# Schaudge/cellranger

Measured on AMD Instinct MI355X. Metric: M reads/sec barcode-correct+UMI-count, higher is better.
Workload: dtype u32/u64 integer keys; f64 posterior

## Files before the change

### cellranger_amd/csrc/dedup.hip

```cpp
#include "block_utils.h"
#include "common.h"

int cr_scan_small(crgpu_ctx *ctx, uint32_t *d_data, uint64_t n, uint32_t *d_total_out);
int cr_partition_by_owner(crgpu_ctx *ctx, const uint64_t *d_in, uint64_t *d_out, uint64_t n, uint32_t sh_bc,
                          uint32_t n_ranks, const uint32_t *bounds, uint64_t *counts_out);

#define NONE32 0xFFFFFFFFu

struct crgpu_counts {
    uint64_t n_triplets = 0, n_molecules = 0;
    uint32_t *d_bc = nullptr, *d_feature = nullptr, *d_count = nullptr;
    uint64_t *d_mkeys = nullptr;
    uint32_t *d_mreads = nullptr;
    uint32_t *d_corr_reads = nullptr;
    uint32_t *d_filt_reads = nullptr;
    int32_t *d_mprobe = nullptr;
    uint32_t *d_back = nullptr;
    uint32_t n_back = 0;
    uint32_t n_canon = 0;
    KeyLayout layout;
    bool pt_valid = false;
    uint32_t pt_n_probes = 0;
    uint64_t n_pt = 0;
    uint32_t *d_pt_bc = nullptr, *d_pt_probe = nullptr, *d_pt_count = nullptr;
// ... 512 lines not shown
        }
#undef CR_BUILD_KEYS
        CR_HIP(ctx, hipGetLastError());
    }
    unsigned long long h = 0;
    CR_TRY(crgpu_memcpy_d2h(ctx, &h, d_n, sizeof(h)));
    if (d_vals_out) {
        uint32_t stalled = 0;
        CR_TRY(crgpu_memcpy_d2h(ctx, &stalled, d_lb_abort, sizeof(stalled)));
        if (stalled) {
            ctx->ghist.valid = false;
            return cr_fail(ctx, CRGPU_EHIP, "crgpu_build_keys: the look-back of the order-preserving compaction stalled (watchdog); "
                                            "nothing was hung, the keys of this call are incomplete");
        }
    }
    if (d_fwd) {
        uint32_t unknown = 0;
        CR_TRY(crgpu_memcpy_d2h(ctx, &unknown, d_unknown, sizeof(unknown)));
        if (unknown) {
            ctx->ghist.valid = false;
            return cr_fail(ctx, CRGPU_ESTATE, "crgpu_build_keys: %u records carry a barcode that has no read in the VALID / CORRECTED tables "
                           "(CRGPU_OPT_DENSE_BARCODE_KEYS needs the tables of the whole well before the first key is built)", unknown);
        }
    }
    *n_keys_out = h;
    ctx->ghist.n = append ? n_before + h : h;
    return CRGPU_OK;
}

extern "C" int crgpu_build_keys_dev(crgpu_ctx *ctx, const crgpu_records *recs, uint64_t *d_keys_out,
                                    uint64_t *n_keys_out) {
    if (!ctx) return CRGPU_EINVAL;
    CR_ENTER(ctx);
    return build_keys_impl(ctx, recs, d_keys_out, nullptr, n_keys_out);
}

extern "C" int crgpu_partition_keys_dev(crgpu_ctx *ctx, const uint64_t *d_keys, uint64_t n, uint32_t n_ranks,
                                        const uint32_t *bounds, uint64_t *d_keys_out, uint64_t *counts_out) {
    if (!ctx || !counts_out) return CRGPU_EINVAL;
    CR_ENTER(ctx);
    CR_REQUIRE(ctx, ctx->layout.set, CRGPU_ESTATE, "crgpu_partition_keys: call crgpu_set_key_layout first");
    CR_REQUIRE(ctx, n == 0 || (d_keys && d_keys_out), CRGPU_EINVAL, "crgpu_partition_keys: NULL buffer");
    cr_invalidate(ctx);
    CR_TRY(cr_dense_ensure(ctx));
    return cr_partition_by_owner(ctx, d_keys, d_keys_out, n, ctx->layout.sh_bc(), n_ranks, bounds, counts_out);
}

extern "C" int crgpu_balanced_bounds(crgpu_ctx *ctx, uint32_t n_ranks, uint32_t *bounds_out) {
    if (!ctx || !bounds_out) return CRGPU_EINVAL;
    CR_ENTER(ctx);
    CR_REQUIRE(ctx, ctx->canon_set, CRGPU_ESTATE, "crgpu_balanced_bounds: no whitelist set");
    CR_REQUIRE(ctx, n_ranks >= 1 && n_ranks <= 256, CRGPU_EINVAL, "crgpu_balanced_bounds: n_ranks must be 1..256");
    const uint32_t W = ctx->n_canon;
    std::vector<uint64_t> tot(W, 0);
    std::vector<uint32_t> tmp(W);
    for (int l = 0; l < CRGPU_MAX_LIB; l++) {
        if (!ctx->wl[l].set) continue;
        for (int which = 0; which < 2; which++) {
            CR_TRY(crgpu_memcpy_d2h(ctx, tmp.data(), which ? ctx->wl[l].d_corrected : ctx->wl[l].d_valid, sizeof(uint32_t) * W));
            for (uint32_t r = 0; r < W; r++) tot[r] += tmp[r];
        }
    }
    uint64_t total = 0;
    for (uint32_t r = 0; r < W; r++) total += tot[r];
    bounds_out[0] = 0;
    uint64_t acc = 0;
    uint32_t r = 0;
    for (uint32_t k = 1; k < n_ranks; k++) {
        const uint64_t want = total * k / n_ranks;
        while (r < W && acc + tot[r] <= want) acc += tot[r++];
        bounds_out[k] = r;
    }
    bounds_out[n_ranks] = W;
    return CRGPU_OK;
}

#define CP_BLOCK 256
#ifndef CP_ITEMS
#define CP_ITEMS 8
#endif
#define CP_ROUND (CP_BLOCK * CP_ITEMS)
#define CP_WAVES (CP_BLOCK / 64)

template <typename Flag>
__global__ __launch_bounds__(CP_BLOCK) void k_cp_count(Flag flag, uint64_t n, uint64_t tile, uint32_t *__restrict__ block_counts) {
    __shared__ uint32_t ws[CP_WAVES];
    const uint64_t lo = (uint64_t)blockIdx.x * tile;
    const uint64_t hi = lo + tile < n ? lo + tile : n;
    uint32_t c = 0;
    for (uint64_t base = lo; base < hi; base += CP_ROUND) {
        bool f[CP_ITEMS];
#pragma unroll
        for (int j = 0; j < CP_ITEMS; j++) {
            const uint64_t i = base + (uint64_t)j * CP_BLOCK + threadIdx.x;
            f[j] = flag(i < hi ? i : hi - 1);
        }
#pragma unroll
        for (int j = 0; j < CP_ITEMS; j++) {
            const uint64_t i = base + (uint64_t)j * CP_BLOCK + threadIdx.x;
            c += (f[j] && i < hi) ? 1u : 0u;
        }
    }
#pragma unroll
    for (int d = 32; d >= 1; d >>= 1) c += __shfl_xor(c, d);
    if ((threadIdx.x & 63u) == 0) ws[threadIdx.x >> 6] = c;
    __syncthreads();
    if (threadIdx.x == 0) {
        uint32_t t = 0;
        for (int w = 0; w < CP_WAVES; w++) t += ws[w];
        block_counts[blockIdx.x] = t;
    }
}

template <typename Flag, typename Emit>
__global__ __launch_bounds__(CP_BLOCK) void k_cp_write(Flag flag, Emit emit, uint64_t n, uint64_t tile,
                                                       const uint32_t *__restrict__ block_offs) {
    __shared__ uint32_t ws[CP_ITEMS * CP_WAVES];
    __shared__ uint32_t round_total;
    const uint32_t lane = threadIdx.x & 63u, wave = threadIdx.x >> 6;
    const uint64_t lo = (uint64_t)blockIdx.x * tile;
    const uint64_t hi = lo + tile < n ? lo + tile : n;
    uint32_t run = block_offs[blockIdx.x];
    for (uint64_t base = lo; base < hi; base += CP_ROUND) {
        bool f[CP_ITEMS];
        typename Emit::Pre pre[CP_ITEMS];
#pragma unroll
        for (int j = 0; j < CP_ITEMS; j++) {
            const uint64_t i = base + (uint64_t)j * CP_BLOCK + threadIdx.x;
            f[j] = flag(i < hi ? i : hi - 1);
            pre[j] = emit.pre(i < hi ? i : hi - 1);
        }
        uint32_t below[CP_ITEMS];
#pragma unroll
        for (int j = 0; j < CP_ITEMS; j++) {
            const uint64_t i = base + (uint64_t)j * CP_BLOCK + threadIdx.x;
            f[j] = f[j] && i < hi;
            const unsigned long long m = __ballot(f[j]);
            below[j] = (uint32_t)__popcll(m & ((1ull << lane) - 1ull));
            if (lane == 0) ws[j * CP_WAVES + wave] = (uint32_t)__popcll(m);
        }
        __syncthreads();
        if (threadIdx.x < CP_ITEMS * CP_WAVES) {
            const uint32_t v = ws[threadIdx.x];
            uint32_t x = v;
#pragma unroll
            for (int d = 1; d < CP_ITEMS * CP_WAVES; d <<= 1) {
                const uint32_t y = __shfl_up(x, d);
                if (threadIdx.x >= (uint32_t)d) x += y;
            }
            ws[threadIdx.x] = x - v;
            if (threadIdx.x == CP_ITEMS * CP_WAVES - 1) round_total = x;
        }
        __syncthreads();
#pragma unroll
        for (int j = 0; j < CP_ITEMS; j++) {
            const uint64_t i = base + (uint64_t)j * CP_BLOCK + threadIdx.x;
            if (f[j]) emit(i, run + ws[j * CP_WAVES + wave] + below[j], pre[j]);
        }
        run += round_total;
        __syncthreads();
    }
}

static uint32_t cp_blocks(uint64_t n, uint64_t *tile_out) {
    uint64_t nb = (n + CP_ROUND * 4 - 1) / (CP_ROUND * 4);
    if (nb < 1) nb = 1;
    if (nb > 4096) nb = 4096;
    uint64_t tile = (n + nb - 1) / nb;
    tile = (tile + CP_ROUND - 1) / CP_ROUND * CP_ROUND;
    nb = (n + tile - 1) / tile;
    if (nb < 1) nb = 1;
    *tile_out = tile;
    return (uint32_t)nb;
}

template <typename Flag, typename Emit>
static int compact(crgpu_ctx *ctx, Flag flag, Emit emit, uint64_t n, uint32_t *d_block, uint32_t *d_total_out) {
    uint64_t tile;
    const uint32_t nb = cp_blocks(n, &tile);
    hipLaunchKernelGGL(k_cp_count<Flag>, dim3(nb), dim3(CP_BLOCK), 0, ctx->stream, flag, n, tile, d_block);
    CR_TRY(cr_scan_small(ctx, d_block, nb, d_total_out));
    hipLaunchKernelGGL((k_cp_write<Flag, Emit>), dim3(nb), dim3(CP_BLOCK), 0, ctx->stream, flag, emit, n, tile, d_block);
    CR_HIP(ctx, hipGetLastError());
    return CRGPU_OK;
}

#define ST_CORRECTED 1u
#define ST_LOW 2u
__device__ __forceinline__ uint32_t st_inc1(uint32_t s) { return s >> 2; }
__device__ __forceinline__ void st_or(uint16_t *st, uint64_t k, uint32_t bits) {
    atomicOr(reinterpret_cast<uint32_t *>(st) + (k >> 1), bits << (16u * (uint32_t)(k & 1u)));
}
__device__ __forceinline__ void move_reads(uint32_t *corr, uint16_t *st, uint32_t *inc_all, uint32_t *minidx, uint64_t k,
                                           uint32_t target, uint32_t my_cnt) {
    corr[k] = target;
    st_or(st, k, ST_CORRECTED);
    atomicAdd(reinterpret_cast<uint32_t *>(st) + (target >> 1), 4u << (16u * (target & 1u)));
    atomicAdd(&inc_all[target], my_cnt);
    atomicMin(&minidx[target], (uint32_t)k);
}
__device__ __forceinline__ uint32_t rep_source(uint32_t min_raw, uint32_t K, uint32_t sK) {
    return (min_raw != 0xFFFFFFFFu && (min_raw < K || (sK & ST_CORRECTED))) ? min_raw : 0xFFFFFFFFu;
}

struct TargetFilter {
    const uint8_t *on_target;
    uint32_t n_features, sh_feat, bits_feat;
    uint64_t min_reads;
    __device__ __forceinline__ bool filtered(uint64_t key, uint32_t read_count, bool low) const {
        if (!min_reads) return false;
        const uint32_t f = (uint32_t)((key >> sh_feat) & lowmask(bits_feat));
        return f < n_features && on_target[f] != 0 && (uint64_t)read_count < min_reads && !low;
    }
};
struct MolFlag {
    const uint16_t *st;
    __device__ __forceinline__ bool operator()(uint64_t k) const {
        const uint32_t s = st[k];
        const bool landed = !(s & ST_CORRECTED) | (st_inc1(s) > 0u);
        return landed & !(s & ST_LOW);
    }
};
struct MolFlagTargeted {
    const uint16_t *st;
    const uint64_t *ukey;
    const uint32_t *upos, *inc_all;
    uint64_t n_keys, n_dist;
    TargetFilter tf;
    __device__ __forceinline__ bool operator()(uint64_t k) const {
        const uint32_t s = st[k];
        const bool landed = !(s & ST_CORRECTED) | (st_inc1(s) > 0u);
        if (!landed || (s & ST_LOW)) return false;
        const uint32_t end = k + 1 < n_dist ? upos[k + 1] : (uint32_t)n_keys;
        const uint32_t rc = ((s & ST_CORRECTED) ? 0u : end - upos[k]) + (st_inc1(s) ? inc_all[k] : 0u);
        return !tf.filtered(ukey[k], rc, false);
    }
};
struct EmitMol {
    const uint64_t *ukey;
    const uint32_t *upos, *inc_all, *minidx;
    const uint16_t *st;
    uint64_t n_keys, n_dist;
    uint64_t *mkeys;
    uint32_t *mreads;
    const uint32_t *rep_read = nullptr;
    const int32_t *probe = nullptr;
    int32_t *mprobe = nullptr;
    struct Pre {
        uint64_t key;
        uint32_t p0, p1, s;
    };
    __device__ __forceinline__ Pre pre(uint64_t k) const {
        Pre p;
        p.key = ukey[k];
        p.p0 = upos[k];
        p.p1 = upos[k + 1 < n_dist ? k + 1 : k];
        p.s = st[k];
        return p;
    }
    __device__ __forceinline__ Pre pre_own(uint64_t k) const {
        Pre p;
        p.key = ukey[k];
        p.p0 = upos[k];
        p.p1 = 0u;
        p.s = st[k];
        return p;
    }
    __device__ __forceinline__ void operator()(uint64_t k, uint32_t o, const Pre &p) const {
        uint32_t inc = 0u, mi = NONE32;
        if (st_inc1(p.s)) {
            inc = inc_all[k];
            mi = rep_source(minidx[k], (uint32_t)k, p.s);
        }
        const uint64_t bit = (mi != NONE32 ? ukey[mi] : p.key) & 1ull;
        mkeys[o] = (p.key & ~1ull) | bit;
        const uint32_t end = k + 1 < n_dist ? p.p1 : (uint32_t)n_keys;
        const uint32_t cnt = end - p.p0;
        mreads[o] = ((p.s & ST_CORRECTED) ? 0u : cnt) + inc;
        if (mprobe) mprobe[o] = probe[rep_read[mi != NONE32 ? mi : (uint32_t)k]];
    }
};

__device__ __forceinline__ bool rl_is_head(uint64_t key, uint64_t &carry_key, bool &carry_valid, uint32_t shift, uint32_t lane) {
    uint64_t left = __shfl_up(key, 1);
    if (lane == 0) left = carry_key;
    const bool head = (lane == 0 && !carry_valid) || (key >> shift) != (left >> shift);
    carry_key = __shfl(key, 63);
    carry_valid = true;
    return head;
}

__global__ __launch_bounds__(CP_BLOCK) void k_rl_count(const uint64_t *__restrict__ keys, const uint32_t shift, const uint64_t n,
                                                       const uint64_t tile, uint32_t *__restrict__ block_counts) {
    __shared__ uint32_t ws[CP_WAVES];
    const uint32_t lane = threadIdx.x & 63u, wave = threadIdx.x >> 6;
    const uint64_t lo = (uint64_t)blockIdx.x * tile;
    const uint64_t hi = lo + tile < n ? lo + tile : n;
    uint32_t c = 0;
    for (uint64_t base = lo; base < hi; base += CP_ROUND) {
        uint64_t key[CP_ITEMS];
        const uint64_t w0 = base + (uint64_t)wave * (64u * CP_ITEMS);
        const uint64_t wb = w0 > 0 ? (w0 - 1 < n ? w0 - 1 : n - 1) : 0;
        uint64_t carry_key = keys[wb];
        bool carry_valid = w0 > 0;
#pragma unroll
        for (int j = 0; j < CP_ITEMS; j++) {
            const uint64_t i = w0 + (uint64_t)j * 64 + lane;
            key[j] = keys[i < hi ? i : hi - 1];
        }
#pragma unroll
        for (int j = 0; j < CP_ITEMS; j++) {
            const uint64_t i = w0 + (uint64_t)j * 64 + lane;
            const bool head = rl_is_head(key[j], carry_key, carry_valid, shift, lane);
            c += (head && i < hi) ? 1u : 0u;
        }
    }
#pragma unroll
    for (int d = 32; d >= 1; d >>= 1) c += __shfl_xor(c, d);
    if (lane == 0) ws[wave] = c;
    __syncthreads();
    if (threadIdx.x == 0) {
        uint32_t t = 0;
        for (int w = 0; w < CP_WAVES; w++) t += ws[w];
        block_counts[blockIdx.x] = t;
    }
}

__global__ __launch_bounds__(CP_BLOCK) void k_rl_write(const uint64_t *__restrict__ keys, const uint32_t shift, const uint64_t n,
                                                       const uint64_t tile, const uint32_t *__restrict__ block_offs,
                                                       uint64_t *__restrict__ ukey, uint32_t *__restrict__ upos) {
    __shared__ uint32_t ws[CP_ITEMS * CP_WAVES];
    __shared__ uint32_t round_total;
    const uint32_t lane = threadIdx.x & 63u, wave = threadIdx.x >> 6;
    const uint64_t lo = (uint64_t)blockIdx.x * tile;
    const uint64_t hi = lo + tile < n ? lo + tile : n;
    uint32_t run = block_offs[blockIdx.x];
    for (uint64_t base = lo; base < hi; base += CP_ROUND) {
        uint64_t key[CP_ITEMS];
        bool f[CP_ITEMS];
        uint32_t below[CP_ITEMS];
        const uint64_t w0 = base + (uint64_t)wave * (64u * CP_ITEMS);
        const uint64_t wb = w0 > 0 ? (w0 - 1 < n ? w0 - 1 : n - 1) : 0;
        uint64_t carry_key = keys[wb];
        bool carry_valid = w0 > 0;
#pragma unroll
        for (int j = 0; j < CP_ITEMS; j++) {
            const uint64_t i = w0 + (uint64_t)j * 64 + lane;
            key[j] = keys[i < hi ? i : hi - 1];
        }
#pragma unroll
        for (int j = 0; j < CP_ITEMS; j++) {
            const uint64_t i = w0 + (uint64_t)j * 64 + lane;
            f[j] = rl_is_head(key[j], carry_key, carry_valid, shift, lane) && i < hi;
            const unsigned long long m = __ballot(f[j]);
            below[j] = (uint32_t)__popcll(m & ((1ull << lane) - 1ull));
            if (lane == 0) ws[wave * CP_ITEMS + j] = (uint32_t)__popcll(m);
        }
        __syncthreads();
        if (threadIdx.x < CP_ITEMS * CP_WAVES) {
            const uint32_t v = ws[threadIdx.x];
            uint32_t x = v;
#pragma unroll
            for (int d = 1; d < CP_ITEMS * CP_WAVES; d <<= 1) {
                const uint32_t y = __shfl_up(x, d);
                if (threadIdx.x >= (uint32_t)d) x += y;
            }
            ws[threadIdx.x] = x - v;
            if (threadIdx.x == CP_ITEMS * CP_WAVES - 1) round_total = x;
        }
        __syncthreads();
#pragma unroll
        for (int j = 0; j < CP_ITEMS; j++)
            if (f[j]) {
                const uint32_t o = run + ws[wave * CP_ITEMS + j] + below[j];
                ukey[o] = key[j];
                upos[o] = (uint32_t)(w0 + (uint64_t)j * 64 + lane);
            }
        run += round_total;
        __syncthreads();
    }
}

static int run_lengths(crgpu_ctx *ctx, const uint64_t *keys, uint32_t shift, uint64_t n, uint64_t *ukey, uint32_t *upos,
                       uint32_t *d_block, uint32_t *d_total_out, bool counts_ready = false) {
    uint64_t tile;
    const uint32_t nb = cp_blocks(n, &tile);
    if (!counts_ready)
        hipLaunchKernelGGL(k_rl_count, dim3(nb), dim3(CP_BLOCK), 0, ctx->stream, keys, shift, n, tile, d_block);
    else
        ctx->rl_counts_from_finish++;
    CR_TRY(cr_scan_small(ctx, d_block, nb, d_total_out));
    hipLaunchKernelGGL(k_rl_write, dim3(nb), dim3(CP_BLOCK), 0, ctx->stream, keys, shift, n, tile, d_block, ukey, upos);
    CR_HIP(ctx, hipGetLastError());
    return CRGPU_OK;
}

struct MtCarry {
    uint64_t prefix;
    bool has_mol;
    bool valid;
};

template <typename Flag>
__device__ __forceinline__ MtCarry mt_carry_from_memory(const Flag &flag, const uint64_t *__restrict__ ukey, uint32_t sh_feat,
                                                        uint64_t nd, uint64_t i0) {
    MtCarry c{0ull, false, false};
    if (i0 == 0 || i0 >= nd) return c;
    c.valid = true;
    uint64_t p = i0 - 1;
    c.prefix = ukey[p] >> sh_feat;
    c.has_mol = flag(p);
    while (!c.has_mol && p > 0) {
        p--;
        if ((ukey[p] >> sh_feat) != c.prefix) break;
        c.has_mol = flag(p);
    }
    return c;
}

__device__ __forceinline__ bool mt_opens_triplet(bool is_mol, uint64_t key, uint32_t sh_feat, uint32_t lane, MtCarry &carry) {
    const uint64_t prefix = key >> sh_feat;
    const uint64_t left = __shfl_up(prefix, 1);
    const unsigned long long starts = __ballot(lane == 0 || prefix != left), mols = __ballot(is_mol);
    const unsigned long long upto = ~0ull >> (63u - lane);
    const uint32_t rs = 63u - (uint32_t)__clzll((long long)(starts & upto));
    const unsigned long long between = (upto >> 1) & ~((1ull << rs) - 1ull);
    const uint64_t prefix0 = __shfl(prefix, 0);
    const bool carried = carry.valid && carry.prefix == prefix0 && carry.has_mol;
    const bool open = (mols & between) == 0ull && !(rs == 0u && carried);
    const uint32_t rs_last = 63u - (uint32_t)__clzll((long long)starts);
    const bool last_has = (mols >> rs_last) != 0ull || (rs_last == 0u && carried);
    carry.prefix = __shfl(prefix, 63);
    carry.has_mol = last_has;
    carry.valid = true;
    return is_mol && open;
}

#define MT_WAVE_SPAN (64u * CP_ITEMS)
template <typename Flag>
__global__ __launch_bounds__(CP_BLOCK) void k_mt_count(const Flag flag, const uint64_t *__restrict__ ukey, const uint32_t sh_feat,
                                                       const uint64_t nd, const uint64_t tile, uint32_t *__restrict__ mol_counts,
                                                       uint32_t *__restrict__ head_counts) {
    __shared__ uint32_t ws[2 * CP_WAVES];
    const uint32_t lane = threadIdx.x & 63u, wave = threadIdx.x >> 6;
    const uint64_t lo = (uint64_t)blockIdx.x * tile;
    const uint64_t hi = lo + tile < nd ? lo + tile : nd;
    uint32_t cm = 0, ch = 0;
    for (uint64_t base = lo; base < hi; base += CP_ROUND) {
        bool f[CP_ITEMS];
        uint64_t key[CP_ITEMS];
        const uint64_t w0 = base + (uint64_t)wave * MT_WAVE_SPAN;
#pragma unroll
        for (int j = 0; j < CP_ITEMS; j++) {
            const uint64_t i = w0 + (uint64_t)j * 64 + lane;
            const uint64_t ic = i < hi ? i : hi - 1;
            f[j] = flag(ic);
            key[j] = ukey[ic];
        }
        MtCarry carry = mt_carry_from_memory(flag, ukey, sh_feat, nd, w0);
#pragma unroll
        for (int j = 0; j < CP_ITEMS; j++) {
            const uint64_t i = w0 + (uint64_t)j * 64 + lane;
            const bool m = f[j] && i < hi;
            const bool h = mt_opens_triplet(m, key[j], sh_feat, lane, carry);
            cm += m ? 1u : 0u;
            ch += h ? 1u : 0u;
        }
    }
#pragma unroll
    for (int d = 32; d >= 1; d >>= 1) {
        cm += __shfl_xor(cm, d);
        ch += __shfl_xor(ch, d);
    }
    if (lane == 0) {
        ws[wave] = cm;
        ws[CP_WAVES + wave] = ch;
    }
    __syncthreads();
    if (threadIdx.x == 0) {
        uint32_t tm = 0, th = 0;
        for (int w = 0; w < CP_WAVES; w++) {
            tm += ws[w];
            th += ws[CP_WAVES + w];
        }
        mol_counts[blockIdx.x] = tm;
        head_counts[blockIdx.x] = th;
    }
}

template <typename Flag>
__global__ __launch_bounds__(CP_BLOCK) void k_mt_write(const Flag flag, const EmitMol emit, const uint32_t sh_bc, const uint32_t sh_feat,
                                                       const uint32_t bits_feat, const uint64_t nd, const uint64_t tile,
                                                       const uint32_t *__restrict__ mol_offs, const uint32_t *__restrict__ head_offs,
                                                       uint32_t *__restrict__ tbc, uint32_t *__restrict__ tfeat,
                                                       uint32_t *__restrict__ tpos, const uint32_t *__restrict__ back) {
    __shared__ uint32_t ws[CP_ITEMS * CP_WAVES];
    __shared__ uint32_t round_total;
    const uint32_t lane = threadIdx.x & 63u, wave = threadIdx.x >> 6;
    const uint64_t lo = (uint64_t)blockIdx.x * tile;
    const uint64_t hi = lo + tile < nd ? lo + tile : nd;
    uint32_t run_m = mol_offs[blockIdx.x], run_h = head_offs[blockIdx.x];
    for (uint64_t base = lo; base < hi; base += CP_ROUND) {
        bool f[CP_ITEMS], h[CP_ITEMS];
        EmitMol::Pre pre[CP_ITEMS];
        const uint64_t w0 = base + (uint64_t)wave * MT_WAVE_SPAN;
#pragma unroll
        for (int j = 0; j < CP_ITEMS; j++) {
            const uint64_t i = w0 + (uint64_t)j * 64 + lane;
            const uint64_t ic = i < hi ? i : hi - 1;
            f[j] = flag(ic);
            pre[j] = emit.pre_own(ic);
        }
        {
            const uint64_t il = w0 + (uint64_t)MT_WAVE_SPAN;
            uint32_t after = emit.upos[il < nd ? il : nd - 1];
#pragma unroll
            for (int j = CP_ITEMS - 1; j >= 0; j--) {
                uint32_t nx = __shfl_down(pre[j].p0, 1);
                if (lane == 63u) nx = after;
                pre[j].p1 = nx;
                after = __shfl(pre[j].p0, 0);
            }
        }
        MtCarry carry = mt_carry_from_memory(flag, emit.ukey, sh_feat, nd, w0);
        uint32_t below_m[CP_ITEMS], below_h[CP_ITEMS];
#pragma unroll
        for (int j = 0; j < CP_ITEMS; j++) {
            const uint64_t i = w0 + (uint64_t)j * 64 + lane;
            f[j] = f[j] && i < hi;
            h[j] = mt_opens_triplet(f[j], pre[j].key, sh_feat, lane, carry);
            const unsigned long long mm = __ballot(f[j]), mh = __ballot(h[j]);
            const unsigned long long lt = (1ull << lane) - 1ull;
            below_m[j] = (uint32_t)__popcll(mm & lt);
            below_h[j] = (uint32_t)__popcll(mh & lt);
            if (lane == 0) ws[wave * CP_ITEMS + j] = (uint32_t)__popcll(mm) | ((uint32_t)__popcll(mh) << 16);
        }
        __syncthreads();
        if (threadIdx.x < CP_ITEMS * CP_WAVES) {
            const uint32_t v = ws[threadIdx.x];
            uint32_t x = v;
#pragma unroll
            for (int d = 1; d < CP_ITEMS * CP_WAVES; d <<= 1) {
                const uint32_t y = __shfl_up(x, d);
                if (threadIdx.x >= (uint32_t)d) x += y;
            }
            ws[threadIdx.x] = x - v;
            if (threadIdx.x == CP_ITEMS * CP_WAVES - 1) round_total = x;
        }
        __syncthreads();
#pragma unroll
        for (int j = 0; j < CP_ITEMS; j++)
            if (f[j]) {
                const uint64_t i = w0 + (uint64_t)j * 64 + lane;
                const uint32_t w = ws[wave * CP_ITEMS + j];
                const uint32_t o = run_m + (w & 0xFFFFu) + below_m[j];
                emit(i, o, pre[j]);
                if (h[j]) {
                    const uint32_t t = run_h + (w >> 16) + below_h[j];
                    const uint32_t bcf = (uint32_t)(pre[j].key >> sh_bc);
                    tbc[t] = back ? back[bcf] : bcf;
                    tfeat[t] = (uint32_t)((pre[j].key >> sh_feat) & lowmask(bits_feat));
                    tpos[t] = o;
                }
            }
        run_m += round_total & 0xFFFFu;
        run_h += round_total >> 16;
        __syncthreads();
    }
}

__global__ __launch_bounds__(256) void k_trip_counts(const uint32_t *__restrict__ tpos, uint64_t nt, uint64_t nm,
                                                     uint32_t *__restrict__ cnt) {
    const uint64_t stride = (uint64_t)gridDim.x * blockDim.x;
    for (uint64_t t = (uint64_t)blockIdx.x * blockDim.x + threadIdx.x; t < nt; t += stride)
        cnt[t] = (t + 1 < nt ? tpos[t + 1] : (uint32_t)nm) - tpos[t];
}

__device__ __forceinline__ void segment_bounds(const uint64_t *__restrict__ ukey, uint64_t nd, uint64_t k, uint32_t shift,
                                               uint64_t &s, uint64_t &e) {
    const uint64_t pre = ukey[k] >> shift;
    uint64_t lo = k, step = 1;
    while (lo >= step && (ukey[lo - step] >> shift) == pre) {
        lo -= step;
        step <<= 1;
    }
    uint64_t a = lo >= step ? lo - step + 1 : 0, b = lo;
    while (a < b) {
        const uint64_t mid = (a + b) >> 1;
        if ((ukey[mid] >> shift) == pre) b = mid; else a = mid + 1;
    }
    s = a;
    uint64_t hi = k;
    step = 1;
    while (hi + step < nd && (ukey[hi + step] >> shift) == pre) {
        hi += step;
        step <<= 1;
    }
    a = hi;
    b = hi + step < nd ? hi + step - 1 : nd - 1;
    while (a < b) {
        const uint64_t mid = (a + b + 1) >> 1;
        if ((ukey[mid] >> shift) == pre) a = mid; else b = mid - 1;
    }
    e = a + 1;
}

__device__ __forceinline__ uint32_t run_count(const uint32_t *__restrict__ upos, uint64_t nd, uint64_t n_keys, uint64_t k) {
    const uint32_t end = k + 1 < nd ? upos[k + 1] : (uint32_t)n_keys;
    return end - upos[k];
}

#include "umi_correct.h"

__device__ __forceinline__ uint64_t group_id(const KL &kl, uint64_t key) {
    const uint64_t umi = (key >> kl.sh_umi) & lowmask(kl.bits_umi);
    const uint64_t lib = (key >> kl.sh_lib) & lowmask(kl.bits_lib + kl.bits_ulen);
    const uint64_t bc = key >> kl.sh_bc;
    return ((bc << (kl.bits_lib + kl.bits_ulen)) | lib) << kl.bits_umi | umi;
}
__device__ __forceinline__ uint32_t group_hash(uint64_t g) {
    g ^= g >> 33;
    g *= 0xff51afd7ed558ccdull;
    g ^= g >> 33;
    g *= 0xc4ceb9fe1a85ec53ull;
    g ^= g >> 33;
    return (uint32_t)g;
}

#define LF_TILE 8192u
#define LF_ENTRY_BITS 18u
#define LF_WORDS (1u << (LF_ENTRY_BITS - 4u))
__device__ __forceinline__ uint64_t mix64(uint64_t g) {
    g ^= g >> 33;
    g *= 0xff51afd7ed558ccdull;
    g ^= g >> 33;
    g *= 0xc4ceb9fe1a85ec53ull;
    g ^= g >> 33;
    return g;
}
#define LF_THREADS 1024u
#define LF_BATCH 4
#define LS_HASH_BITS 32u
__device__ __forceinline__ void lf_note(uint32_t *bm, uint32_t e) {
    const uint32_t sh = (e & 15u) * 2u;
    const uint32_t old = atomicOr(&bm[e >> 4], 1u << sh);
    if ((old >> sh) & 1u) atomicOr(&bm[e >> 4], 2u << sh);
}
__device__ __forceinline__ bool lf_again(const uint32_t *bm, uint32_t e) { return (bm[e >> 4] >> ((e & 15u) * 2u + 1u)) & 1u; }
__global__ __launch_bounds__(LF_THREADS) void k_group_candidates(const KL kl, const uint64_t *__restrict__ ukey, uint64_t nd,
                                                                 uint8_t *__restrict__ cand) {
// ... 563 lines not shown
                                   s_in_tmp ? ht_b.as<uint32_t>() : h_b.as<uint32_t>(),
                                   s_in_tmp ? vt_b.as<uint32_t>() : v_b.as<uint32_t>(), n_cand, nd, vbits, ukey, upos, n_keys, st);
                CR_HIP(ctx, hipGetLastError());
            }
        }
        CR_TRY(fork.join());
    }

    const TargetFilter tf{ctx->d_on_target, ctx->n_target_features, L.sh_feat(), L.bits_feat, ctx->d_on_target ? ctx->target_min_reads : 0};
    CrFork fork2(ctx);
    DevBuf rep_b, packed_b;
    const bool want_probe = vals && pr.d_probe;
    if (vals) CR_TRY(dmalloc(ctx, rep_b, nd * sizeof(uint32_t)));
    if (want_probe) {
        CrTimer t(ctx, CRGPU_T_DEDUP);
        hipLaunchKernelGGL(k_rep_read, dim3(cr_grid(nd, 256)), dim3(256), 0, ctx->stream, keys, vals, upos, nd, n_keys,
                           rep_b.as<uint32_t>());
        CR_HIP(ctx, hipGetLastError());
    }
    if (vals && CrFork::enabled(ctx, nd)) {
        CR_TRY(fork2.mark());
        CR_TRY(fork2.side(fork2.t0));
    }
    const uint32_t side_wgs = fork2.on_side ? 256u * 6u : 256u * 8u;
    if (vals) {
        CrTimer t(ctx, CRGPU_T_DEDUP);
        if (!want_probe)
            hipLaunchKernelGGL(k_rep_read, dim3(cr_grid(nd, 256, side_wgs)), dim3(256), 0, ctx->stream, keys, vals, upos, nd, n_keys,
                               rep_b.as<uint32_t>());
        if (pr.packed_out) CR_HIP(ctx, hipMemsetAsync(pr.packed_out, 0, pr.n_reads * sizeof(DupRec), ctx->stream));
        const bool pack8 = !pr.packed_out && kl.bits_umi <= 24u;
        if (!pr.packed_out) {
            const uint64_t bytes = pr.n_reads * (pack8 ? sizeof(DupRec8) : sizeof(DupRec));
            CR_TRY(dmalloc(ctx, packed_b, bytes));
            CR_HIP(ctx, hipMemsetAsync(packed_b.p, 0, bytes, ctx->stream));
        }
        DupRec *packed = pr.packed_out ? pr.packed_out : packed_b.as<DupRec>();
        if (pack8)
            hipLaunchKernelGGL(k_per_read<true>, dim3(cr_grid(nd, 256, side_wgs)), dim3(256), 0, ctx->stream, kl, ukey, vals, upos, nd, n_keys,
                               corr, inc_all, st, minidx, rep_b.as<uint32_t>(), (void *)packed, tf);
        else
            hipLaunchKernelGGL(k_per_read<false>, dim3(cr_grid(nd, 256, side_wgs)), dim3(256), 0, ctx->stream, kl, ukey, vals, upos, nd, n_keys,
                               corr, inc_all, st, minidx, rep_b.as<uint32_t>(), (void *)packed, tf);
        if (!pr.packed_out) {
            if (pack8)
                hipLaunchKernelGGL(k_unpack_dupinfo<true>, dim3(cr_grid(pr.n_reads, 256, side_wgs)), dim3(256), 0, ctx->stream,
                                   (const void *)packed, pr.n_reads, pr.out_umi, pr.out_cnt, pr.out_flags);
            else
                hipLaunchKernelGGL(k_unpack_dupinfo<false>, dim3(cr_grid(pr.n_reads, 256, side_wgs)), dim3(256), 0, ctx->stream,
                                   (const void *)packed, pr.n_reads, pr.out_umi, pr.out_cnt, pr.out_flags);
        }
        CR_HIP(ctx, hipGetLastError());
    }
    fork2.pause();

    DevBuf mkeys_b, mreads_b, tpos_b;
    CR_TRY(dmalloc(ctx, mkeys_b, nd * sizeof(uint64_t)));
    CR_TRY(dmalloc(ctx, mreads_b, nd * sizeof(uint32_t)));
    uint32_t nm32 = 0, nt32 = 0;
    if (want_probe) CR_TRY(cr_pool_alloc(ctx, (void **)&res->d_mprobe, nd * sizeof(int32_t)));
    CR_TRY(dmalloc(ctx, tpos_b, (nd + 1) * sizeof(uint32_t)));
    CR_TRY(cr_pool_alloc(ctx, (void **)&res->d_bc, nd * sizeof(uint32_t)));
    CR_TRY(cr_pool_alloc(ctx, (void **)&res->d_feature, nd * sizeof(uint32_t)));
    uint32_t *d_heads = d_block + 4096;
    uint32_t *d_total_h = ctx->d_scalars + 17;
    {
        CrTimer t(ctx, CRGPU_T_DEDUP);
        EmitMol emit{ukey, upos, inc_all, minidx, st, n_keys, nd, mkeys_b.as<uint64_t>(), mreads_b.as<uint32_t>()};
        if (want_probe) {
            emit.rep_read = rep_b.as<uint32_t>();
            emit.probe = pr.d_probe;
            emit.mprobe = res->d_mprobe;
        }
        uint64_t tile;
        const uint32_t nb = cp_blocks(nd, &tile);
        const MolFlagTargeted flag_t{st, ukey, upos, inc_all, n_keys, nd, tf};
        const MolFlag flag_p{st};
        if (tf.min_reads)
            hipLaunchKernelGGL(k_mt_count<MolFlagTargeted>, dim3(nb), dim3(CP_BLOCK), 0, ctx->stream, flag_t, ukey, L.sh_feat(), nd,
                               tile, d_block, d_heads);
        else
            hipLaunchKernelGGL(k_mt_count<MolFlag>, dim3(nb), dim3(CP_BLOCK), 0, ctx->stream, flag_p, ukey, L.sh_feat(), nd, tile,
                               d_block, d_heads);
        CR_TRY(cr_scan_small(ctx, d_block, nb, d_total));
        CR_TRY(cr_scan_small(ctx, d_heads, nb, d_total_h));
        if (tf.min_reads)
            hipLaunchKernelGGL(k_mt_write<MolFlagTargeted>, dim3(nb), dim3(CP_BLOCK), 0, ctx->stream, flag_t, emit, L.sh_bc(),
                               L.sh_feat(), L.bits_feat, nd, tile, d_block, d_heads, res->d_bc, res->d_feature, tpos_b.as<uint32_t>(),
                               res->d_back);
        else
            hipLaunchKernelGGL(k_mt_write<MolFlag>, dim3(nb), dim3(CP_BLOCK), 0, ctx->stream, flag_p, emit, L.sh_bc(), L.sh_feat(),
                               L.bits_feat, nd, tile, d_block, d_heads, res->d_bc, res->d_feature, tpos_b.as<uint32_t>(), res->d_back);
        CR_HIP(ctx, hipGetLastError());
    }
    CR_TRY(read_u32(ctx, d_total, &nm32));
    CR_TRY(read_u32(ctx, d_total_h, &nt32));
    const uint64_t nm = nm32;

    if (pr.summary) {
        const size_t bytes = ((size_t)1 << L.bits_lib) * ctx->n_canon * sizeof(uint32_t);
        CR_TRY(cr_pool_alloc(ctx, (void **)&res->d_corr_reads, bytes));
        CrTimer t(ctx, CRGPU_T_DEDUP);
        CR_HIP(ctx, hipMemsetAsync(res->d_corr_reads, 0, bytes, ctx->stream));
        hipLaunchKernelGGL(k_corrected_reads, dim3(cr_grid(nd, 256)), dim3(256), 0, ctx->stream, kl, ukey, upos, nd, n_keys, st,
                           ctx->n_canon, res->d_corr_reads, res->d_back);
        if (tf.min_reads) {
            CR_TRY(cr_pool_alloc(ctx, (void **)&res->d_filt_reads, bytes));
            CR_HIP(ctx, hipMemsetAsync(res->d_filt_reads, 0, bytes, ctx->stream));
            hipLaunchKernelGGL(k_filtered_reads, dim3(cr_grid(nd, 256)), dim3(256), 0, ctx->stream, kl, ukey, upos, nd, n_keys, st,
                               inc_all, tf, ctx->n_canon, res->d_filt_reads, res->d_back);
        }
        CR_HIP(ctx, hipGetLastError());
    }

    const uint64_t nt = nt32;
    CR_TRY(cr_pool_alloc(ctx, (void **)&res->d_count, nt * sizeof(uint32_t)));
    if (nt) {
        CrTimer t(ctx, CRGPU_T_DEDUP);
        hipLaunchKernelGGL(k_trip_counts, dim3(cr_grid(nt, 256)), dim3(256), 0, ctx->stream, tpos_b.as<uint32_t>(), nt, nm, res->d_count);
        CR_HIP(ctx, hipGetLastError());
    }
    CR_TRY(fork2.join());
    res->n_triplets = nt;
    res->n_molecules = nm;
    res->d_mkeys = (uint64_t *)mkeys_b.p;
    res->d_mreads = (uint32_t *)mreads_b.p;
    mkeys_b.p = nullptr;
    mreads_b.p = nullptr;
    guard.armed = false;
    *out = res;
    return CRGPU_OK;
}

extern "C" int crgpu_count_keys_dev(crgpu_ctx *ctx, uint64_t *d_keys_inout, uint64_t n_keys, crgpu_counts **out) {
    if (!ctx) return CRGPU_EINVAL;
    CR_ENTER(ctx);
    PerRead pr;
    pr.summary = ctx->barcode_summary_on;
    return count_keys_impl(ctx, d_keys_inout, n_keys, out, pr);
}

extern "C" int crgpu_count_records_dev(crgpu_ctx *ctx, const crgpu_records *recs, crgpu_counts **out,
                                       uint32_t *d_processed_umi_out, uint32_t *d_read_count_out, uint8_t *d_dupflags_out) {
    if (!ctx || !recs || !out) return CRGPU_EINVAL;
    CR_ENTER(ctx);
    *out = nullptr;
    CR_REQUIRE(ctx, recs->n <= 0x7FFFFFFFull, CRGPU_ERANGE, "crgpu_count_records: at most 2^31-1 records per call");
    const uint64_t n = recs->n;
    DevBuf keys_b, vals_b;
    CR_TRY(dmalloc(ctx, keys_b, n * sizeof(uint64_t)));
    CR_TRY(dmalloc(ctx, vals_b, n * sizeof(uint32_t)));
    uint64_t n_keys = 0;
    CR_TRY(build_keys_impl(ctx, recs, keys_b.as<uint64_t>(), vals_b.as<uint32_t>(), &n_keys));
    PerRead pr;
    pr.summary = true;
    pr.n_reads = n;
    pr.d_vals = vals_b.as<uint32_t>();
    pr.out_umi = d_processed_umi_out;
    pr.out_cnt = d_read_count_out;
    pr.out_flags = d_dupflags_out;
    pr.d_probe = recs->d_probe_idx;
    if (n_keys == 0) {
        if (d_processed_umi_out) CR_HIP(ctx, hipMemsetAsync(d_processed_umi_out, 0, n * sizeof(uint32_t), ctx->stream));
        if (d_read_count_out) CR_HIP(ctx, hipMemsetAsync(d_read_count_out, 0, n * sizeof(uint32_t), ctx->stream));
        if (d_dupflags_out) CR_HIP(ctx, hipMemsetAsync(d_dupflags_out, 0, n, ctx->stream));
    }
    return count_keys_impl(ctx, keys_b.as<uint64_t>(), n_keys, out, pr);
}

__global__ __launch_bounds__(256) void k_iota_u32(uint32_t *p, uint64_t n) {
    const uint64_t stride = (uint64_t)gridDim.x * blockDim.x;
    for (uint64_t i = (uint64_t)blockIdx.x * blockDim.x + threadIdx.x; i < n; i += stride) p[i] = (uint32_t)i;
}
__global__ __launch_bounds__(256) void k_scatter_dupinfo(const DupRec *__restrict__ rec, const uint32_t *__restrict__ ordinal,
                                                         uint64_t n_keys, uint32_t *__restrict__ out_umi,
// ... 771 lines not shown
```

### cellranger_amd/csrc/sort.hip

```cpp
#include <cstdlib>
#include <cstring>
#include <type_traits>
#include <vector>

#include "block_utils.h"
#include <algorithm>

#include "common.h"

#ifdef SORT_NT_IN
#define SORT_LOAD_IN(p) __builtin_nontemporal_load(p)
#else
#define SORT_LOAD_IN(p) (*(p))
#endif
#ifdef SORT_NT_OUT
#define SORT_STORE_OUT(v, p) __builtin_nontemporal_store((v), (p))
#else
#define SORT_STORE_OUT(v, p) (*(p) = (v))
#endif
#ifndef SORT_BLOCK
#define SORT_BLOCK 1024
#endif
#ifndef SORT_ITEMS
#define SORT_ITEMS 16
#endif
#ifndef SORT_ITEMS_KV64
#define SORT_ITEMS_KV64 10
#endif
#define SORT_WAVES (SORT_BLOCK / 64)
#define RADIX_BITS 8
#define RADIX 256
#ifndef SORT_LB
#define SORT_LB 8
#endif
#ifndef SORT_MAX_BLOCKS
#define SORT_MAX_BLOCKS 1024
#endif
#define OR_MAX_LOW_BITS 16u

__global__ __launch_bounds__(1024) void k_scan_small(uint32_t *__restrict__ data, uint64_t n,
                                                     uint32_t *__restrict__ total_out) {
    __shared__ uint32_t wave_sums[16];
    __shared__ uint32_t carry_s;
    const uint32_t tid = threadIdx.x, lane = tid & 63u, wave = tid >> 6;
    if (tid == 0) carry_s = 0;
    __syncthreads();
    for (uint64_t base = 0; base < n; base += 1024) {
        const uint64_t i = base + tid;
        const uint32_t v = i < n ? data[i] : 0u;
        uint32_t x = v;
#pragma unroll
        for (int d = 1; d < 64; d <<= 1) {
            const uint32_t y = __shfl_up(x, d);
            if (lane >= (uint32_t)d) x += y;
        }
        if (lane == 63) wave_sums[wave] = x;
        __syncthreads();
        uint32_t wpre = 0, tot = 0;
        for (uint32_t w = 0; w < 16; w++) {
            const uint32_t t = wave_sums[w];
            if (w < wave) wpre += t;
            tot += t;
        }
        const uint32_t carry = carry_s;
        if (i < n) data[i] = carry + wpre + x - v;
        __syncthreads();
        if (tid == 0) carry_s = carry + tot;
        __syncthreads();
    }
    if (tid == 0 && total_out) *total_out = carry_s;
}

int cr_scan_small(crgpu_ctx *ctx, uint32_t *d_data, uint64_t n, uint32_t *d_total_out) {
    CrTimer t(ctx, CRGPU_T_SCAN);
    hipLaunchKernelGGL(k_scan_small, dim3(1), dim3(1024), 0, ctx->stream, d_data, n, d_total_out);
    CR_HIP(ctx, hipGetLastError());
    return CRGPU_OK;
}

struct RadixDigit {
    uint32_t shift, mask;
    template <typename K>
    __device__ __forceinline__ uint32_t operator()(K key, uint32_t = 0u) const {
        return (uint32_t)(key >> shift) & mask;
    }
};
struct OwnerDiv {
    uint32_t shift, width;
    template <typename K>
    __device__ __forceinline__ uint32_t operator()(K key, uint32_t = 0u) const {
        return (uint32_t)((uint64_t)key >> shift) / width;
    }
};
struct OwnerBounds {
    uint32_t shift, width;
    const uint32_t *bounds;
    template <typename K>
    __device__ __forceinline__ uint32_t operator()(K key, uint32_t = 0u) const {
        const uint32_t v = (uint32_t)((uint64_t)key >> shift);
        uint32_t lo = 0, hi = width;
        while (lo + 1 < hi) {
            const uint32_t mid = (lo + hi) >> 1;
            if (bounds[mid] <= v) lo = mid; else hi = mid;
        }
        return lo;
    }
};

template <typename K, bool HAS_VALS>
struct SortCfg {
    static constexpr int ITEMS = (sizeof(K) == 8 && HAS_VALS) ? SORT_ITEMS_KV64 : SORT_ITEMS;
    static constexpr uint32_t CHUNK = SORT_BLOCK * ITEMS;
    static constexpr size_t lds_bytes(int bits) {
        return (size_t)CHUNK * (sizeof(K) + (HAS_VALS ? 4 : 0)) + (size_t)SORT_WAVES * (1u << bits) * 2 +
               2 * (size_t)(1u << bits) * 4 + SORT_WAVES * 4 + 16;
    }
};

template <typename K, typename DIG, int BITS>
__global__ __launch_bounds__(SORT_BLOCK) void k_radix_hist(const K *__restrict__ keys, const uint32_t *__restrict__ vals,
                                                           uint64_t n, uint64_t tile, DIG dig,
                                                           uint32_t *__restrict__ block_hist, uint32_t n_blocks) {
    constexpr uint32_t RADIX_T = 1u << BITS;
    __shared__ uint32_t h[RADIX_T];
    if (threadIdx.x < RADIX_T) h[threadIdx.x] = 0;
    __syncthreads();
    const uint64_t lo = (uint64_t)blockIdx.x * tile;
    const uint64_t hi = lo + tile < n ? lo + tile : n;
    for (uint64_t i = lo + threadIdx.x; i < hi; i += SORT_BLOCK) atomicAdd(&h[dig(keys[i], vals ? vals[i] : 0u)], 1u);
    __syncthreads();
    if (threadIdx.x < RADIX_T) block_hist[(uint64_t)threadIdx.x * n_blocks + blockIdx.x] = h[threadIdx.x];
}

__global__ __launch_bounds__(256) void k_scan_digits(uint32_t *__restrict__ block_hist, uint32_t n_blocks,
                                                     uint32_t *__restrict__ digit_totals) {
    __shared__ uint32_t lds[8];
    uint32_t *row = block_hist + (uint64_t)blockIdx.x * n_blocks;
    uint32_t carry = 0;
    for (uint32_t base = 0; base < n_blocks; base += 256) {
        const uint32_t i = base + threadIdx.x;
        const uint32_t v = i < n_blocks ? row[i] : 0u;
        uint32_t tot;
        const uint32_t pre = block_excl_scan_256(v, lds, &tot);
        if (i < n_blocks) row[i] = carry + pre;
        carry += tot;
    }
    if (threadIdx.x == 0) digit_totals[blockIdx.x] = carry;
}

#ifdef SORT_PHASE_TIMING
__device__ unsigned long long g_sort_phase[16];
#define SORT_PH(i)                                                          \
    do {                                                                    \
        if (tid == 0) {                                                     \
            const unsigned long long t_ = __builtin_readcyclecounter();     \
            atomicAdd(&g_sort_phase[i], t_ - ph_t);                         \
            ph_t = t_;                                                      \
        }                                                                   \
// ... 1156 lines not shown
```

Measured before the change: 17380.

## Fuse block-offset scan into compaction write kernels and retune small scan

The compaction, run-length and molecule-table write kernels no longer depend on a separate single-block scan launch. Each block now computes its own base offset by summing the preceding block counts with vectorized loads and a block reduction, and the last block writes the total. This removes one or two serial single-block kernel launches per compaction, at the cost of redundant quadratic-ish reads of the counts array across blocks. The standalone small scan is also reshaped to 256 threads with 4 items per thread.

```diff
diff --git a/cellranger_amd/csrc/dedup.hip b/cellranger_amd/csrc/dedup.hip
--- a/cellranger_amd/csrc/dedup.hip
+++ b/cellranger_amd/csrc/dedup.hip
@@ -618,6 +618,26 @@
 #define CP_ROUND (CP_BLOCK * CP_ITEMS)
 #define CP_WAVES (CP_BLOCK / 64)
 
+__device__ __forceinline__ uint32_t cp_block_base(const uint32_t *__restrict__ counts, uint32_t b) {
+    __shared__ uint32_t part[CP_WAVES];
+    uint32_t s = 0;
+    const uint32_t nq = b >> 2;
+    for (uint32_t q = threadIdx.x; q < nq; q += CP_BLOCK) {
+        const uint4 v = reinterpret_cast<const uint4 *>(counts)[q];
+        s += v.x + v.y + v.z + v.w;
+    }
+    if (threadIdx.x < (b & 3u)) s += counts[(nq << 2) + threadIdx.x];
+#pragma unroll
+    for (int d = 32; d >= 1; d >>= 1) s += __shfl_xor(s, d);
+    if ((threadIdx.x & 63u) == 0) part[threadIdx.x >> 6] = s;
+    __syncthreads();
+    uint32_t t = 0;
+#pragma unroll
+    for (int w = 0; w < CP_WAVES; w++) t += part[w];
+    __syncthreads();
+    return t;
+}
+
 template <typename Flag>
 __global__ __launch_bounds__(CP_BLOCK) void k_cp_count(Flag flag, uint64_t n, uint64_t tile, uint32_t *__restrict__ block_counts) {
     __shared__ uint32_t ws[CP_WAVES];
@@ -650,13 +670,13 @@
 
 template <typename Flag, typename Emit>
 __global__ __launch_bounds__(CP_BLOCK) void k_cp_write(Flag flag, Emit emit, uint64_t n, uint64_t tile,
-                                                       const uint32_t *__restrict__ block_offs) {
+                                                       const uint32_t *__restrict__ block_counts, uint32_t *__restrict__ total_out) {
     __shared__ uint32_t ws[CP_ITEMS * CP_WAVES];
     __shared__ uint32_t round_total;
     const uint32_t lane = threadIdx.x & 63u, wave = threadIdx.x >> 6;
     const uint64_t lo = (uint64_t)blockIdx.x * tile;
     const uint64_t hi = lo + tile < n ? lo + tile : n;
-    uint32_t run = block_offs[blockIdx.x];
+    uint32_t run = cp_block_base(block_counts, blockIdx.x);
     for (uint64_t base = lo; base < hi; base += CP_ROUND) {
         bool f[CP_ITEMS];
         typename Emit::Pre pre[CP_ITEMS];
@@ -696,6 +716,7 @@
         run += round_total;
         __syncthreads();
     }
+    if (blockIdx.x == gridDim.x - 1 && threadIdx.x == 0) *total_out = run;
 }
 
 static uint32_t cp_blocks(uint64_t n, uint64_t *tile_out) {
@@ -715,8 +736,7 @@
     uint64_t tile;
     const uint32_t nb = cp_blocks(n, &tile);
     hipLaunchKernelGGL(k_cp_count<Flag>, dim3(nb), dim3(CP_BLOCK), 0, ctx->stream, flag, n, tile, d_block);
-    CR_TRY(cr_scan_small(ctx, d_block, nb, d_total_out));
-    hipLaunchKernelGGL((k_cp_write<Flag, Emit>), dim3(nb), dim3(CP_BLOCK), 0, ctx->stream, flag, emit, n, tile, d_block);
+    hipLaunchKernelGGL((k_cp_write<Flag, Emit>), dim3(nb), dim3(CP_BLOCK), 0, ctx->stream, flag, emit, n, tile, d_block, d_total_out);
     CR_HIP(ctx, hipGetLastError());
     return CRGPU_OK;
 }
@@ -863,14 +883,15 @@
 }
 
 __global__ __launch_bounds__(CP_BLOCK) void k_rl_write(const uint64_t *__restrict__ keys, const uint32_t shift, const uint64_t n,
-                                                       const uint64_t tile, const uint32_t *__restrict__ block_offs,
-                                                       uint64_t *__restrict__ ukey, uint32_t *__restrict__ upos) {
+                                                       const uint64_t tile, const uint32_t *__restrict__ block_counts,
+                                                       uint32_t *__restrict__ total_out, uint64_t *__restrict__ ukey,
+                                                       uint32_t *__restrict__ upos) {
     __shared__ uint32_t ws[CP_ITEMS * CP_WAVES];
     __shared__ uint32_t round_total;
     const uint32_t lane = threadIdx.x & 63u, wave = threadIdx.x >> 6;
     const uint64_t lo = (uint64_t)blockIdx.x * tile;
     const uint64_t hi = lo + tile < n ? lo + tile : n;
-    uint32_t run = block_offs[blockIdx.x];
+    uint32_t run = cp_block_base(block_counts, blockIdx.x);
     for (uint64_t base = lo; base < hi; base += CP_ROUND) {
         uint64_t key[CP_ITEMS];
         bool f[CP_ITEMS];
@@ -915,6 +936,7 @@
         run += round_total;
         __syncthreads();
     }
+    if (blockIdx.x == gridDim.x - 1 && threadIdx.x == 0) *total_out = run;
 }
 
 static int run_lengths(crgpu_ctx *ctx, const uint64_t *keys, uint32_t shift, uint64_t n, uint64_t *ukey, uint32_t *upos,
@@ -925,8 +947,7 @@
         hipLaunchKernelGGL(k_rl_count, dim3(nb), dim3(CP_BLOCK), 0, ctx->stream, keys, shift, n, tile, d_block);
     else
         ctx->rl_counts_from_finish++;
-    CR_TRY(cr_scan_small(ctx, d_block, nb, d_total_out));
-    hipLaunchKernelGGL(k_rl_write, dim3(nb), dim3(CP_BLOCK), 0, ctx->stream, keys, shift, n, tile, d_block, ukey, upos);
+    hipLaunchKernelGGL(k_rl_write, dim3(nb), dim3(CP_BLOCK), 0, ctx->stream, keys, shift, n, tile, d_block, d_total_out, ukey, upos);
     CR_HIP(ctx, hipGetLastError());
     return CRGPU_OK;
 }
@@ -1027,7 +1048,8 @@
 template <typename Flag>
 __global__ __launch_bounds__(CP_BLOCK) void k_mt_write(const Flag flag, const EmitMol emit, const uint32_t sh_bc, const uint32_t sh_feat,
                                                        const uint32_t bits_feat, const uint64_t nd, const uint64_t tile,
-                                                       const uint32_t *__restrict__ mol_offs, const uint32_t *__restrict__ head_offs,
+                                                       const uint32_t *__restrict__ mol_counts, const uint32_t *__restrict__ head_counts,
+                                                       uint32_t *__restrict__ mol_total, uint32_t *__restrict__ head_total,
                                                        uint32_t *__restrict__ tbc, uint32_t *__restrict__ tfeat,
                                                        uint32_t *__restrict__ tpos, const uint32_t *__restrict__ back) {
     __shared__ uint32_t ws[CP_ITEMS * CP_WAVES];
@@ -1035,7 +1057,7 @@
     const uint32_t lane = threadIdx.x & 63u, wave = threadIdx.x >> 6;
     const uint64_t lo = (uint64_t)blockIdx.x * tile;
     const uint64_t hi = lo + tile < nd ? lo + tile : nd;
-    uint32_t run_m = mol_offs[blockIdx.x], run_h = head_offs[blockIdx.x];
+    uint32_t run_m = cp_block_base(mol_counts, blockIdx.x), run_h = cp_block_base(head_counts, blockIdx.x);
     for (uint64_t base = lo; base < hi; base += CP_ROUND) {
         bool f[CP_ITEMS], h[CP_ITEMS];
         EmitMol::Pre pre[CP_ITEMS];
@@ -1102,6 +1124,10 @@
         run_m += round_total & 0xFFFFu;
         run_h += round_total >> 16;
         __syncthreads();
+    }
+    if (blockIdx.x == gridDim.x - 1 && threadIdx.x == 0) {
+        *mol_total = run_m;
+        *head_total = run_h;
     }
 }
 
@@ -1831,15 +1857,14 @@
         else
             hipLaunchKernelGGL(k_mt_count<MolFlag>, dim3(nb), dim3(CP_BLOCK), 0, ctx->stream, flag_p, ukey, L.sh_feat(), nd, tile,
                                d_block, d_heads);
-        CR_TRY(cr_scan_small(ctx, d_block, nb, d_total));
-        CR_TRY(cr_scan_small(ctx, d_heads, nb, d_total_h));
         if (tf.min_reads)
             hipLaunchKernelGGL(k_mt_write<MolFlagTargeted>, dim3(nb), dim3(CP_BLOCK), 0, ctx->stream, flag_t, emit, L.sh_bc(),
-                               L.sh_feat(), L.bits_feat, nd, tile, d_block, d_heads, res->d_bc, res->d_feature, tpos_b.as<uint32_t>(),
+                               L.sh_feat(), L.bits_feat, nd, tile, d_block, d_heads, d_total, d_total_h, res->d_bc, res->d_feature, tpos_b.as<uint32_t>(),
                                res->d_back);
         else
             hipLaunchKernelGGL(k_mt_write<MolFlag>, dim3(nb), dim3(CP_BLOCK), 0, ctx->stream, flag_p, emit, L.sh_bc(), L.sh_feat(),
-                               L.bits_feat, nd, tile, d_block, d_heads, res->d_bc, res->d_feature, tpos_b.as<uint32_t>(), res->d_back);
+                               L.bits_feat, nd, tile, d_block, d_heads, d_total, d_total_h, res->d_bc, res->d_feature, tpos_b.as<uint32_t>(),
+                               res->d_back);
         CR_HIP(ctx, hipGetLastError());
     }
     CR_TRY(read_u32(ctx, d_total, &nm32));
diff --git a/cellranger_amd/csrc/sort.hip b/cellranger_amd/csrc/sort.hip
--- a/cellranger_amd/csrc/sort.hip
+++ b/cellranger_amd/csrc/sort.hip
@@ -38,32 +38,52 @@
 #endif
 #define OR_MAX_LOW_BITS 16u
 
-__global__ __launch_bounds__(1024) void k_scan_small(uint32_t *__restrict__ data, uint64_t n,
-                                                     uint32_t *__restrict__ total_out) {
-    __shared__ uint32_t wave_sums[16];
+#define SCAN_SMALL_THREADS 256u
+#define SCAN_SMALL_ITEMS 4u
+#define SCAN_SMALL_ROUND (SCAN_SMALL_THREADS * SCAN_SMALL_ITEMS)
+#define SCAN_SMALL_RUNS (SCAN_SMALL_ROUND / 64u)
+__global__ __launch_bounds__(SCAN_SMALL_THREADS) void k_scan_small(uint32_t *__restrict__ data, uint64_t n,
+                                                                   uint32_t *__restrict__ total_out) {
+    __shared__ uint32_t run_sums[SCAN_SMALL_RUNS];
     __shared__ uint32_t carry_s;
     const uint32_t tid = threadIdx.x, lane = tid & 63u, wave = tid >> 6;
     if (tid == 0) carry_s = 0;
     __syncthreads();
-    for (uint64_t base = 0; base < n; base += 1024) {
-        const uint64_t i = base + tid;
-        const uint32_t v = i < n ? data[i] : 0u;
-        uint32_t x = v;
+    for (uint64_t base = 0; base < n; base += SCAN_SMALL_ROUND) {
+        uint32_t v[SCAN_SMALL_ITEMS], x[SCAN_SMALL_ITEMS];
+#pragma unroll
+        for (uint32_t j = 0; j < SCAN_SMALL_ITEMS; j++) {
+            const uint64_t i = base + j * SCAN_SMALL_THREADS + tid;
+            v[j] = i < n ? data[i] : 0u;
+            x[j] = v[j];
+        }
 #pragma unroll
         for (int d = 1; d < 64; d <<= 1) {
-            const uint32_t y = __shfl_up(x, d);
-            if (lane >= (uint32_t)d) x += y;
-        }
-        if (lane == 63) wave_sums[wave] = x;
-        __syncthreads();
-        uint32_t wpre = 0, tot = 0;
-        for (uint32_t w = 0; w < 16; w++) {
-            const uint32_t t = wave_sums[w];
-            if (w < wave) wpre += t;
+#pragma unroll
+            for (uint32_t j = 0; j < SCAN_SMALL_ITEMS; j++) {
+                const uint32_t y = __shfl_up(x[j], d);
+                if (lane >= (uint32_t)d) x[j] += y;
+            }
+        }
+        if (lane == 63) {
+#pragma unroll
+            for (uint32_t j = 0; j < SCAN_SMALL_ITEMS; j++) run_sums[j * (SCAN_SMALL_THREADS / 64u) + wave] = x[j];
+        }
+        __syncthreads();
+        uint32_t pre[SCAN_SMALL_ITEMS] = {0u, 0u, 0u, 0u}, tot = 0;
+        for (uint32_t w = 0; w < SCAN_SMALL_RUNS; w++) {
+            const uint32_t t = run_sums[w];
+#pragma unroll
+            for (uint32_t j = 0; j < SCAN_SMALL_ITEMS; j++)
+                if (w < j * (SCAN_SMALL_THREADS / 64u) + wave) pre[j] += t;
             tot += t;
         }
         const uint32_t carry = carry_s;
-        if (i < n) data[i] = carry + wpre + x - v;
+#pragma unroll
+        for (uint32_t j = 0; j < SCAN_SMALL_ITEMS; j++) {
+            const uint64_t i = base + j * SCAN_SMALL_THREADS + tid;
+            if (i < n) data[i] = carry + pre[j] + x[j] - v[j];
+        }
         __syncthreads();
         if (tid == 0) carry_s = carry + tot;
         __syncthreads();
@@ -73,7 +93,7 @@
 
 int cr_scan_small(crgpu_ctx *ctx, uint32_t *d_data, uint64_t n, uint32_t *d_total_out) {
     CrTimer t(ctx, CRGPU_T_SCAN);
-    hipLaunchKernelGGL(k_scan_small, dim3(1), dim3(1024), 0, ctx->stream, d_data, n, d_total_out);
+    hipLaunchKernelGGL(k_scan_small, dim3(1), dim3(SCAN_SMALL_THREADS), 0, ctx->stream, d_data, n, d_total_out);
     CR_HIP(ctx, hipGetLastError());
     return CRGPU_OK;
 }
```

Result: no change. 17260 (-0.7%).
